# facebookresearch/vilbert-multi-task

Hardware: NVIDIA H100
Metric: (region,token) pairs/sec fwd+bwd, bert_base_6layer_6conect (higher is better)
Workload: dtype fp16

## Files before the change

include/vilbert_b200.h:

```cpp
#ifndef VILBERT_B200_H_
#define VILBERT_B200_H_

#include <stddef.h>
#include <stdint.h>

#ifdef __cplusplus
extern "C" {
#endif

typedef int vb_status;
enum {
  VB_OK = 0,
  VB_ERR_INVALID = 1,
  VB_ERR_UNSUPPORTED = 2,
  VB_ERR_CUDA = 3
};

enum { VB_ACT_NONE = 0, VB_ACT_GELU = 1, VB_ACT_RELU = 2, VB_ACT_DGELU = 3 };

typedef struct vb_dropout_site {
  const uint32_t* step;
  uint32_t site;
  float p;
} vb_dropout_site;
// ... 29 lines not shown
  int64_t ld_out_bf16;
  void* out_pre;
  int64_t ld_out_pre;
  int32_t atomic_out;
  float* out_colsum;
  vb_dropout_site dropout;
  int32_t split_k;
  int32_t block_n;
  int32_t max_ctas;
  void* dbg_timeline;
  int32_t a_fp16, b_fp16, out_fp16;
  const void* A_lo;
  const void* B_lo;
  void* out_lo;
  void* out_b16;
} vb_gemm_args;

vb_status vb_gemm_bf16(const vb_gemm_args* args, void* stream);

vb_status vb_gemm_plan(const vb_gemm_args* args, int32_t sm_count, int32_t* block_n, int32_t* split_k);

typedef struct vb_attn_args {
  int32_t B, H, Nq, Nk, D;
  const void* Q; int64_t ldq;
  const void* K; int64_t ldk;
  const void* V; int64_t ldv;
  const float* mask;
  float scale;
  void* O; int64_t ldo;
  float* lse;
  const void* dO; int64_t lddo;
  void* dQ; int64_t lddq;
  void* dK; int64_t lddk;
  void* dV; int64_t lddv;
  float* delta;
// ... 263 lines not shown
```

vilbert-multi-task_b200/_lib.py:

```python
import ctypes as C
import os
import re
from collections import namedtuple

import torch

_HERE = os.path.dirname(os.path.abspath(__file__))
LIB_PATH = os.path.join(_HERE, "libvilbert_b200.so")
HEADER_PATH = os.path.normpath(os.path.join(_HERE, "..", "include", "vilbert_b200.h"))


class VBError(RuntimeError):
    pass


class DropoutSite(C.Structure):

    _fields_ = [("step", C.c_void_p), ("site", C.c_uint32), ("p", C.c_float)]


class Dropout(DropoutSite):

    _fields_ = [("row_map", C.c_void_p)]

# ... 4 lines not shown
        ("M", C.c_int32), ("N", C.c_int32), ("K", C.c_int32),
        ("A", C.c_void_p), ("lda", C.c_int64), ("a_mn_major", C.c_int32),
        ("B", C.c_void_p), ("ldb", C.c_int64), ("b_mn_major", C.c_int32),
        ("alpha", C.c_float),
        ("bias", C.c_void_p),
        ("residual", C.c_void_p), ("ld_res", C.c_int64),
        ("aux", C.c_void_p), ("ld_aux", C.c_int64),
        ("act", C.c_int32),
        ("out_f32", C.c_void_p), ("ld_out_f32", C.c_int64),
        ("out_bf16", C.c_void_p), ("ld_out_bf16", C.c_int64),
        ("out_pre", C.c_void_p), ("ld_out_pre", C.c_int64),
        ("atomic_out", C.c_int32), ("out_colsum", C.c_void_p), ("dropout", DropoutSite), ("split_k", C.c_int32), ("block_n", C.c_int32), ("max_ctas", C.c_int32),
        ("dbg_timeline", C.c_void_p),
        ("a_fp16", C.c_int32), ("b_fp16", C.c_int32), ("out_fp16", C.c_int32),
        ("A_lo", C.c_void_p), ("B_lo", C.c_void_p), ("out_lo", C.c_void_p), ("out_b16", C.c_void_p),
    ]


class AttnArgs(C.Structure):

    _fields_ = [
        ("B", C.c_int32), ("H", C.c_int32), ("Nq", C.c_int32), ("Nk", C.c_int32), ("D", C.c_int32),
        ("Q", C.c_void_p), ("ldq", C.c_int64), ("K", C.c_void_p), ("ldk", C.c_int64), ("V", C.c_void_p), ("ldv", C.c_int64),
        ("mask", C.c_void_p), ("scale", C.c_float),
        ("O", C.c_void_p), ("ldo", C.c_int64), ("lse", C.c_void_p),
        ("dO", C.c_void_p), ("lddo", C.c_int64), ("dQ", C.c_void_p), ("lddq", C.c_int64),
        ("dK", C.c_void_p), ("lddk", C.c_int64), ("dV", C.c_void_p), ("lddv", C.c_int64),
        ("delta", C.c_void_p),
        ("dbias_q", C.c_void_p), ("dbias_k", C.c_void_p), ("dbias_v", C.c_void_p),
        ("dropout", DropoutSite),
# ... 131 lines not shown
```

vilbert-multi-task_b200/csrc/vb_gemm.cu:

```cuda
#include <cuda.h>
#include <cuda_bf16.h>
#include <cuda_runtime.h>
#include <stdint.h>

#include <type_traits>

#include "vb_internal.h"
#include "vb_ptx.cuh"

namespace vb {

constexpr int BM = 128;
constexpr int BK = 64;
constexpr int UK = 16;
constexpr int CONSUMER_WARPS = 8;
constexpr int GEMM_THREADS = 128 + CONSUMER_WARPS * 32;
constexpr int EPI_ROWS = 16;
constexpr int EPI_PS = EPI_ROWS / 4;
constexpr int STAGING_BYTES_PER_WARP = EPI_ROWS * 32 * 4;
__device__ __forceinline__ int stg_off(int row, int col) { return row * 32 + ((((col >> 2) ^ (row & 7)) << 2) | (col & 3)); }

template <int BN>
struct GemmCfg {
  static constexpr int A_BYTES = BM * BK * 2;
// ... 212 lines not shown
  }
  wgmma_commit();
}

template <int NR>
__device__ __forceinline__ void stage_chunk(const float (&d)[NR], int c4, float* stg, int lane) {
  const int r0 = lane >> 2, c0 = 2 * (lane & 3);
#pragma unroll
  for (int ii = 0; ii < 4; ++ii) {
    const int i = c4 * 4 + ii;
    *reinterpret_cast<float2*>(stg + stg_off(r0, ii * 8 + c0)) = make_float2(d[4 * i], d[4 * i + 1]);
    *reinterpret_cast<float2*>(stg + stg_off(r0 + 8, ii * 8 + c0)) = make_float2(d[4 * i + 2], d[4 * i + 3]);
  }
}

template <int BN, int EPI, int OUT16>
__global__ void __launch_bounds__(GEMM_THREADS, 1)
gemm_wgmma_kernel(const __grid_constant__ CUtensorMap tmap_a, const __grid_constant__ CUtensorMap tmap_b,
                  const __grid_constant__ CUtensorMap tmap_a_lo, const __grid_constant__ CUtensorMap tmap_b_lo,
                  const __grid_constant__ GemmKernelParams p) {
  using Cfg = GemmCfg<BN>;
  constexpr int NUM_STAGES = Cfg::NUM_STAGES;

  extern __shared__ __align__(1024) uint8_t smem[];
  if ((smem_u32(smem) & 1023u) != 0) __trap();
  uint8_t* smem_tiles = smem;
  float* staging = reinterpret_cast<float*>(smem + NUM_STAGES * Cfg::STAGE_BYTES);
  uint64_t* bars = reinterpret_cast<uint64_t*>(smem + NUM_STAGES * Cfg::STAGE_BYTES + CONSUMER_WARPS * STAGING_BYTES_PER_WARP);
  uint64_t* full_bar = bars;
  uint64_t* empty_bar = bars + NUM_STAGES;
// ... 12 lines not shown
      mbar_init(smem_u32(&full_bar[s]), 1);
      mbar_init(smem_u32(&empty_bar[s]), CONSUMER_WARPS);
    }
    fence_mbar_init();
  }
  __syncthreads();
  pdl_entry();
  if (threadIdx.x == 0) VB_DBG(1);

  const int group = blockIdx.x;
  const int num_groups = gridDim.x;
  const int total_work = p.num_m_blocks * p.num_n_blocks * p.split_k;

  if (warp_idx < 4) setmaxnreg_dec<40>();
  if (warp_idx == 0) {
    int stage = 0;
    uint32_t phase = 0;
    for (int w = group; w < total_work; w += num_groups) {
      const int split = w % p.split_k;
      const int t2 = w / p.split_k;
      const int m_blk = t2 % p.num_m_blocks;
      const int n_blk = t2 / p.num_m_blocks;
      const int kb0 = split * p.k_blocks_per_split;
      const int kb1 = min(kb0 + p.k_blocks_per_split, p.num_k_blocks);
      auto issue_loads = [&](const CUtensorMap* tma_a, const CUtensorMap* tma_b, int kb) {
        mbar_wait(smem_u32(&empty_bar[stage]), phase ^ 1);
        const uint32_t sa = smem_u32(smem_tiles + stage * Cfg::STAGE_BYTES);
        const uint32_t sb = sa + Cfg::A_BYTES;
        const uint32_t fb = smem_u32(&full_bar[stage]);
        mbar_arrive_expect_tx(fb, Cfg::STAGE_BYTES);
        if (p.a_mn) {
#pragma unroll
          for (int j = 0; j < BM / 64; ++j) tma_load_2d(sa + j * (BK * 128), tma_a, m_blk * BM + j * 64, kb * BK, fb);
        } else {
          tma_load_2d(sa, tma_a, kb * BK, m_blk * BM, fb);
        }
        if (p.b_mn) {
#pragma unroll
          for (int j = 0; j < BN / 64; ++j) tma_load_2d(sb + j * (BK * 128), tma_b, n_blk * BN + j * 64, kb * BK, fb);
        } else {
          tma_load_2d(sb, tma_b, kb * BK, n_blk * BN, fb);
        }
      };
      for (int kbv = kb0; kbv < kb1; ++kbv) {
        if (elect_one()) {
          if (p.npass == 1) {
            issue_loads(&tmap_a, &tmap_b, kbv);
          } else {
            const int ps = kbv / p.real_k_blocks;
            const int sel = p.pass_sel[ps];
            issue_loads((sel & 1) ? &tmap_a_lo : &tmap_a, (sel & 2) ? &tmap_b_lo : &tmap_b, kbv - ps * p.real_k_blocks);
          }
          if (kbv == kb0 && w == group) VB_DBG(2);
        }
        __syncwarp();
        if (++stage == NUM_STAGES) { stage = 0; phase ^= 1; }
      }
    }
  } else if (warp_idx >= 4) {
    setmaxnreg_inc<232>();
    const int cw = warp_idx - 4;
    const int wg = cw >> 2;
    float* stg = staging + cw * (EPI_ROWS * 32);
    const int rr = lane >> 3;
    const int cc = (lane & 7) * 4;
    const uint32_t a_off = wg * (64 * 128);
    auto release = [&](int s) {
      __syncwarp();
      if (lane == 0) mbar_arrive(smem_u32(&empty_bar[s]));
    };
    float acc[BN / 2];
    int stage = 0;
    uint32_t phase = 0;
// ... 26 lines not shown
        case 1: kloop(std::integral_constant<int, 1>{}); break;
        case 2: kloop(std::integral_constant<int, 2>{}); break;
        case 3: kloop(std::integral_constant<int, 3>{}); break;
        case 4: kloop(std::integral_constant<int, 4>{}); break;
        case 5: kloop(std::integral_constant<int, 5>{}); break;
        case 6: kloop(std::integral_constant<int, 6>{}); break;
        default: kloop(std::integral_constant<int, 7>{}); break;
      }
      wgmma_wait<0>();
#pragma unroll
      for (int i = 0; i < BN / 2; ++i) reg_fence(acc[i]);
      if (prev >= 0) release(prev);
      if (w == group && threadIdx.x == 128) VB_DBG(5);

      const int m_base = m_blk * BM + wg * 64 + (cw & 3) * EPI_ROWS;
      const bool rows_full = (m_base + EPI_ROWS <= p.M);
      if (m_base < p.M) {
        constexpr int NC = BN / 32;
#pragma unroll 1
        for (int c = 0; c < NC; ++c) {
          const int n_chunk = n_blk * BN + c * 32;
          if (n_chunk >= p.N) break;
          const bool fast = (EPI != EPI_GENERIC) && p.fast_ok && rows_full && (n_chunk + 32 <= p.N);
          const int n = n_chunk + cc;
          float4 resv[EPI_PS];
          uint2 auxv[EPI_PS];
          float4 b4 = make_float4(0.f, 0.f, 0.f, 0.f);
          if (fast) {
            if (EPI == EPI_F32 && p.residual) {
#pragma unroll
              for (int ps = 0; ps < EPI_PS; ++ps) {
                const float* src = p.residual + (long long)(m_base + ps * 4 + rr) * p.ld_res + n;
                if (p.vec_res) resv[ps] = *reinterpret_cast<const float4*>(src);
                else resv[ps] = make_float4(src[0], src[1], src[2], src[3]);
              }
            }
            if (EPI == EPI_DGELU) {
#pragma unroll
              for (int ps = 0; ps < EPI_PS; ++ps)
                auxv[ps] = *reinterpret_cast<const uint2*>(p.aux + (long long)(m_base + ps * 4 + rr) * p.ld_aux + n);
            }
            if (p.bias) b4 = *reinterpret_cast<const float4*>(p.bias + n);
          }
#pragma unroll
          for (int c2 = 0; c2 < NC; ++c2)
            if (c2 == c) stage_chunk(acc, c2, stg, lane);
          __syncwarp();
          if (EPI == EPI_PARTIAL) {
            if (fast) epi_fast_chunk<EPI, OUT16>(p, stg, m_base + split * p.M, n, rr, cc, resv, auxv, b4);
            else      epi_partial_chunk(p, stg, m_base, n, rr, cc, (long long)split * p.M);
          }
          else if (EPI == EPI_F32 && p.act == VB_ACT_RELU && fast) epi_pool_chunk(p, stg, m_base, n, rr, cc, b4);
          else if (fast) epi_fast_chunk<EPI, OUT16>(p, stg, m_base, n, rr, cc, resv, auxv, b4);
          else           epi_generic_chunk(p, stg, m_base, n, rr, cc);
          __syncwarp();
        }
      }
      if (w == group && threadIdx.x == 128) VB_DBG(6);
    }
  }

  if (threadIdx.x == 0) { VB_DBG(7); VB_DBG_NS(9); }
#undef VB_DBG
#undef VB_DBG_NS
}

typedef CUresult (*PFN_encodeTiled)(CUtensorMap*, CUtensorMapDataType, cuuint32_t, void*, const cuuint64_t*,
                                    const cuuint64_t*, const cuuint32_t*, const cuuint32_t*,
                                    CUtensorMapInterleave, CUtensorMapSwizzle, CUtensorMapL2promotion,
                                    CUtensorMapFloatOOBfill);

static PFN_encodeTiled get_encode_fn() {
  static PFN_encodeTiled fn = nullptr;
// ... 49 lines not shown
      if (out16 == 2) return launch_gemm<BN, EPI_BF16, 2>(tm, p, work, max_ctas, stream);
      if (out16 == 3) return launch_gemm<BN, EPI_BF16, 3>(tm, p, work, max_ctas, stream);
      return launch_gemm<BN, EPI_BF16, 0>(tm, p, work, max_ctas, stream);
    case EPI_GELU:
      if (out16 == 1) return launch_gemm<BN, EPI_GELU, 1>(tm, p, work, max_ctas, stream);
      if (out16 == 2) return launch_gemm<BN, EPI_GELU, 2>(tm, p, work, max_ctas, stream);
      if (out16 == 3) return launch_gemm<BN, EPI_GELU, 3>(tm, p, work, max_ctas, stream);
      return launch_gemm<BN, EPI_GELU, 0>(tm, p, work, max_ctas, stream);
    case EPI_DGELU: return launch_gemm<BN, EPI_DGELU>(tm, p, work, max_ctas, stream);
    case EPI_ATOMIC: return launch_gemm<BN, EPI_ATOMIC>(tm, p, work, max_ctas, stream);
    case EPI_PARTIAL: return launch_gemm<BN, EPI_PARTIAL>(tm, p, work, max_ctas, stream);
    default: return launch_gemm<BN, EPI_GENERIC>(tm, p, work, max_ctas, stream);
  }
}

static inline bool aligned(const void* p, size_t a) { return (reinterpret_cast<uintptr_t>(p) % a) == 0; }

static int choose_config(const vb_gemm_args* a, int max_ctas, int* bn_out, int* split_out) {
  const int num_m = (a->M + BM - 1) / BM;
  const int num_k = (a->K + BK - 1) / BK * (1 + (a->A_lo ? 1 : 0) + (a->B_lo ? 1 : 0));
  if (a->block_n != 0 && a->block_n != 128 && a->block_n != 256) return set_error(VB_ERR_INVALID, "vb_gemm_bf16: block_n must be 0, 128 or 256");
  if (a->split_k > 1 && (!a->atomic_out || a->act != VB_ACT_NONE || a->bias || a->residual || a->out_colsum))
    return set_error(VB_ERR_INVALID, "vb_gemm_bf16: split_k > 1 needs atomic_out and a plain epilogue");
  const bool can_split = a->atomic_out && a->act == VB_ACT_NONE && !a->bias && !a->residual && !a->out_colsum;
  long long epi_base = 9000;
  if (a->atomic_out) epi_base = 3000;
  else if (a->act == VB_ACT_GELU || a->act == VB_ACT_DGELU) epi_base = 4200;
  else if (a->act == VB_ACT_NONE && a->out_f32 && !a->out_bf16) epi_base = a->residual ? 4800 : 3000;
  else if (a->act == VB_ACT_NONE && a->out_bf16 && !a->out_f32) epi_base = 3000;
  int bn = 128, split_k = 1;
  {
    long long best = -1;
    static const int split_cand[] = {1, 2, 3, 4, 5, 6, 8, 10, 12, 16, 24, 32};
// ... 5 lines not shown
      const long long tiles = (long long)num_m * ((a->N + w - 1) / w);
      for (int sc : split_cand) {
        if (a->split_k > 0 && sc != 1) break;
        int sp = a->split_k > 0 ? a->split_k : sc;
        if (sp > 1 && !can_split) break;
        if (sp > num_k) { if (a->split_k > 0) sp = num_k; else break; }
        const long long kps_ = (num_k + sp - 1) / sp;
        sp = (int)((num_k + kps_ - 1) / kps_);
        const long long rounds = (tiles * sp + max_ctas - 1) / max_ctas;
        const long long ml = kps_ * t_kb;
        const long long c = 3000 + rounds * (ml + epi);
        if (best < 0 || c < best) { best = c; bn = w; split_k = sp; }
      }
    }
    if (best < 0) return set_error(VB_ERR_INVALID, "vb_gemm_bf16: no tile configuration for block_n=%d split_k=%d", a->block_n, a->split_k);
  }
  *bn_out = bn; *split_out = split_k;
  return VB_OK;
}

}

extern "C" vb_status vb_gemm_bf16(const vb_gemm_args* a, void* stream_) {
  using namespace vb;
  cudaStream_t stream = static_cast<cudaStream_t>(stream_);
  if (!a) return set_error(VB_ERR_INVALID, "vb_gemm_bf16: null args");
  if (a->M <= 0 || a->N <= 0 || a->K <= 0) return set_error(VB_ERR_INVALID, "vb_gemm_bf16: empty problem %dx%dx%d", a->M, a->N, a->K);
  if (!a->A || !a->B) return set_error(VB_ERR_INVALID, "vb_gemm_bf16: null operand");
  if ((a->lda % 8) || (a->ldb % 8) || !aligned(a->A, 16) || !aligned(a->B, 16))
    return set_error(VB_ERR_INVALID, "vb_gemm_bf16: operands need ld %% 8 == 0 and 16-byte aligned bases (lda=%lld ldb=%lld)",
// ... 8 lines not shown
  if ((a->A_lo && !aligned(a->A_lo, 16)) || (a->B_lo && !aligned(a->B_lo, 16)))
    return set_error(VB_ERR_INVALID, "vb_gemm_bf16: A_lo / B_lo must be 16-byte aligned");
  if ((a->out_lo || a->out_b16) && !a->out_bf16) return set_error(VB_ERR_INVALID, "vb_gemm_bf16: out_lo / out_b16 need out_bf16");
  if ((a->a_fp16 != 0) != (a->b_fp16 != 0))
    return set_error(VB_ERR_UNSUPPORTED, "vb_gemm_bf16: A and B must have the same 16-bit format (wgmma takes one operand type for both)");
  int dev_sms = 0, cc = 0;
  if (int s = vb_device_info(&dev_sms, &cc)) return s;
  if (cc != 90) return set_error(VB_ERR_UNSUPPORTED, "vb_gemm_bf16: needs an sm_90 device (found sm_%d)", cc);

  const int num_m = (a->M + BM - 1) / BM;
  const int real_k = (a->K + BK - 1) / BK;
  const int npass = 1 + (a->A_lo ? 1 : 0) + (a->B_lo ? 1 : 0);
  const int num_k = real_k * npass;
  int max_ctas = a->max_ctas > 0 ? a->max_ctas : dev_sms;

  int bn = 128, split_k = 1;
  if (int st = choose_config(a, max_ctas, &bn, &split_k)) return st;
  const int num_n = (a->N + bn - 1) / bn;
  const int kps = (num_k + split_k - 1) / split_k;

  GemmKernelParams p;
  p.M = a->M; p.N = a->N; p.K = a->K;
  p.num_m_blocks = num_m; p.num_n_blocks = num_n; p.num_k_blocks = num_k;
  p.real_k_blocks = real_k; p.npass = npass;
  p.pass_sel[0] = 0; p.pass_sel[1] = a->A_lo ? 1 : 2; p.pass_sel[2] = 2;
  p.out_fp16 = a->out_fp16 ? 1 : 0;
  p.out_lo = static_cast<__nv_bfloat16*>(a->out_lo);
  p.out_b16 = static_cast<__nv_bfloat16*>(a->out_b16);
  p.split_k = split_k; p.k_blocks_per_split = kps;
  p.alpha = a->alpha;
  p.bias = a->bias;
  p.residual = a->residual; p.ld_res = a->ld_res;
// ... 28 lines not shown
  for (int i = 0; i < 4; ++i) {
    const bool is_a = (i & 1) == 0;
    const void* ptr = is_a ? (i < 2 ? a->A : a->A_lo) : (i < 2 ? a->B : a->B_lo);
    if (!ptr) { tm[i] = tm[i - 2]; continue; }
    if (is_a) {
      if (a->a_mn_major) st = make_tmap(&tm[i], ptr, (uint64_t)a->M, (uint64_t)a->K, (uint64_t)a->lda, 64, BK);
      else               st = make_tmap(&tm[i], ptr, (uint64_t)a->K, (uint64_t)a->M, (uint64_t)a->lda, BK, BM);
    } else {
      if (a->b_mn_major) st = make_tmap(&tm[i], ptr, (uint64_t)a->N, (uint64_t)a->K, (uint64_t)a->ldb, 64, BK);
      else               st = make_tmap(&tm[i], ptr, (uint64_t)a->K, (uint64_t)a->N, (uint64_t)a->ldb, BK, (uint32_t)bn);
    }
    if (st) return st;
  }

  const long long total_work = (long long)num_m * num_n * split_k;
  int epi = EPI_GENERIC;
  const bool no_extra = !a->out_colsum;
  const bool has_drop = p.drop.ctr != nullptr;
  if (a->atomic_out == VB_GEMM_PARTIALS) {
    if (a->act != VB_ACT_NONE || a->bias || a->residual || !no_extra || has_drop || a->split_k != split_k)
      return set_error(VB_ERR_INVALID, "vb_gemm_bf16: VB_GEMM_PARTIALS needs a plain epilogue and split_k as vb_gemm_plan resolves it "
                       "(asked %d, resolved %d)", a->split_k, split_k);
    epi = EPI_PARTIAL; p.fast_ok = p.vec_f32;
  } else if (a->atomic_out) {
    if (a->act == VB_ACT_NONE && !a->bias && !a->residual && no_extra && !has_drop) { epi = EPI_ATOMIC; p.fast_ok = p.vec_f32; }
  } else if (a->act == VB_ACT_GELU) {
    if (a->out_pre && !a->residual && no_extra && !has_drop && (a->out_bf16 || a->out_f32)) {
      epi = EPI_GELU; p.fast_ok = p.vec_pre && (!a->out_bf16 || p.vec_bf16) && (!a->out_f32 || p.vec_f32);
    }
  } else if (a->act == VB_ACT_DGELU) {
    if (a->out_bf16 && !a->out_f32 && !a->residual && !a->bias && !has_drop) { epi = EPI_DGELU; p.fast_ok = p.vec_bf16 && p.vec_aux; }
  } else if (a->act == VB_ACT_RELU) {
    if (a->out_f32 && no_extra && !a->residual && !has_drop) { epi = EPI_F32; p.fast_ok = p.vec_f32 && (!a->out_bf16 || p.vec_bf16); }
  } else if (a->act == VB_ACT_NONE) {
    if (a->out_f32 && !a->out_bf16 && no_extra) { epi = EPI_F32; p.fast_ok = 1; }
    else if (a->out_bf16 && !a->out_f32 && !a->residual && no_extra && !has_drop) { epi = EPI_BF16; p.fast_ok = p.vec_bf16; }
  }
  int out16 = 0;
  if (epi == EPI_BF16 || epi == EPI_GELU) {
    if ((a->out_lo || a->out_b16) && !a->out_fp16) epi = EPI_GENERIC;
    else out16 = a->out_lo ? 3 : (a->out_fp16 ? (a->out_b16 ? 2 : 1) : 0);
  } else if (epi == EPI_DGELU && (a->out_fp16 || a->out_lo || a->out_b16)) {
    epi = EPI_GENERIC;
  }
  if (bn == 256) return launch_gemm_epi<256>(epi, out16, tm, p, total_work, max_ctas, stream);
  return launch_gemm_epi<128>(epi, out16, tm, p, total_work, max_ctas, stream);
}

extern "C" vb_status vb_gemm_plan(const vb_gemm_args* a, int32_t sm_count_, int32_t* block_n, int32_t* split_k) {
  using namespace vb;
  if (!a || !block_n || !split_k) return set_error(VB_ERR_INVALID, "vb_gemm_plan: null argument");
  if (a->M <= 0 || a->N <= 0 || a->K <= 0) return set_error(VB_ERR_INVALID, "vb_gemm_plan: empty problem %dx%dx%d", a->M, a->N, a->K);
  int sms = sm_count_;
  if (sms <= 0) {
    int cc = 0;
    if (int s = vb_device_info(&sms, &cc)) return s;
  }
  const int max_ctas = a->max_ctas > 0 ? a->max_ctas : sms;
  int bn, sp;
  if (int s = choose_config(a, max_ctas, &bn, &sp)) return s;
  *block_n = bn; *split_k = sp;
  return VB_OK;
}
```

vilbert-multi-task_b200/engine.py:

```python
import bisect
import dataclasses
import math
import warnings
import zlib
from collections import Counter, OrderedDict, namedtuple

import torch

from . import _lib as L

F32, BF16, F16, I64 = torch.float32, torch.bfloat16, torch.float16, torch.int64
PRECISIONS = ("fp16", "fp32", "bf16")
BASE_FEATURE_SIZE, BASE_REGION_CLASSES = 2048, 1601
BASE_HEAD_NAMES = ("vil_prediction", "vil_logit", "vil_binary_prediction", "vision_prediction", "vision_logit", "linguisic_prediction",
                   "linguisic_logit")
BASE_BERT_OUT_NAMES = ("sequence_output", "pooled_output")
INPUT_GRAD_NAMES = ("input_imgs", "image_loc")
PACKED_HEADS = ("vil_prediction", "vil_prediction_gqa", "vil_logit", "vil_binary_prediction", "vil_tri_prediction", "vision_logit")
RETRIEVAL_SCORE_HEADS = {"vl": "vil_logit", "pretraining": "seq_relationship_score"}
PACK_REFUSED_CONFIG = ("in_batch_pairs", "fast_mode", "dynamic_attention", "visualization")
PACKED_MASKED_LOGIT = -10000.0


def pack_capacity(count, padded_rows):
# ... 1013 lines not shown
        else:
            self._check_operands((), (A, B, out_bf16))
        g.M, g.N, g.K = M, N, K
        g.A, g.lda, g.a_mn_major = L.arg(A), lda, a_mn
        g.B, g.ldb, g.b_mn_major = L.arg(B), ldb, b_mn
        g.alpha = alpha
        g.bias = L.arg(bias)
        g.residual, g.ld_res = L.arg(residual), ld_res
        g.aux, g.ld_aux = L.arg(aux), ld_aux
        g.act = act
        g.out_f32, g.ld_out_f32 = L.arg(out_f32), ld_of
        g.out_bf16, g.ld_out_bf16 = L.arg(out_bf16), ld_ob
        g.out_pre, g.ld_out_pre = L.arg(out_pre), ld_op
        g.atomic_out, g.split_k, g.block_n, g.max_ctas = atomic, split_k, 0, (0 if fwd else self.spec.bwd_gemm_max_ctas)
        g.out_colsum = L.arg(None if self.det else out_colsum)
        if dropout is not None:
            g.dropout = dropout
        self._keep.append(g)
        if self.det and atomic:
            g.atomic_out, g.split_k = L.VB_GEMM_PARTIALS, 0
            bn, sp = L.C.c_int32(), L.C.c_int32()
            L.check(self.lib.vb_gemm_plan(L.C.byref(g), 132 if self.dev.type != "cuda" else 0, L.C.byref(bn), L.C.byref(sp)),
                    "vb_gemm_plan")
            if sp.value == 1:
                g.atomic_out, g.split_k = 1, 1
                self.emit(self.lib.vb_gemm_bf16, g)
                return
            if ld_of != N:
                raise L.VBError(f"deterministic split-K GEMM needs a dense output (ld {ld_of} != N {N})")
            ws = self.det_ws(sp.value * M * N)
# ... 1858 lines not shown
```

Measured before the change: 12.79 million.

## Add ping-pong warpgroup GEMM schedule with cost-model auto selection

Adds a ping-pong GEMM kernel in which the two consumer warpgroups work on alternate tiles, so one warpgroup's epilogue runs while the other issues WGMMA. Named barriers order the two groups. A cycle-based cost model picks between cooperative and ping-pong per GEMM, and the engine asks for AUTO unless deterministic mode is on. It also prefetches the next chunk's epilogue inputs (residual, aux, bias) during the current chunk. The risks are a poor choice from the hand-fitted cost constants, and extra register pressure from keeping two 64x128 accumulators per warpgroup.

New measurement: 12.77 million, median of 6. About the same (-0.1%).

```diff
diff --git a/include/vilbert_b200.h b/include/vilbert_b200.h
--- a/include/vilbert_b200.h
+++ b/include/vilbert_b200.h
@@ -67,11 +67,15 @@
   const void* B_lo;
   void* out_lo;
   void* out_b16;
+  int32_t schedule;
 } vb_gemm_args;
 
+enum { VB_GEMM_SCHED_COOPERATIVE = 0, VB_GEMM_SCHED_PINGPONG = 1, VB_GEMM_SCHED_AUTO = 2 };
+
 vb_status vb_gemm_bf16(const vb_gemm_args* args, void* stream);
 
 vb_status vb_gemm_plan(const vb_gemm_args* args, int32_t sm_count, int32_t* block_n, int32_t* split_k);
+vb_status vb_gemm_plan_schedule(const vb_gemm_args* args, int32_t sm_count, int32_t* block_n, int32_t* split_k, int32_t* schedule);
 
 typedef struct vb_attn_args {
   int32_t B, H, Nq, Nk, D;
diff --git a/vilbert-multi-task_b200/_lib.py b/vilbert-multi-task_b200/_lib.py
--- a/vilbert-multi-task_b200/_lib.py
+++ b/vilbert-multi-task_b200/_lib.py
@@ -42,6 +42,7 @@
         ("dbg_timeline", C.c_void_p),
         ("a_fp16", C.c_int32), ("b_fp16", C.c_int32), ("out_fp16", C.c_int32),
         ("A_lo", C.c_void_p), ("B_lo", C.c_void_p), ("out_lo", C.c_void_p), ("out_b16", C.c_void_p),
+        ("schedule", C.c_int32),
     ]
 
 
diff --git a/vilbert-multi-task_b200/csrc/vb_gemm.cu b/vilbert-multi-task_b200/csrc/vb_gemm.cu
--- a/vilbert-multi-task_b200/csrc/vb_gemm.cu
+++ b/vilbert-multi-task_b200/csrc/vb_gemm.cu
@@ -250,6 +250,106 @@
   }
 }
 
+template <int BN>
+__device__ __forceinline__ void gemm_produce(const CUtensorMap* tmap_a, const CUtensorMap* tmap_b, const CUtensorMap* tmap_a_lo,
+                                             const CUtensorMap* tmap_b_lo, const GemmKernelParams& p, uint8_t* smem_tiles,
+                                             uint64_t* full_bar, uint64_t* empty_bar, int group, int num_groups, int total_work) {
+  using Cfg = GemmCfg<BN>;
+  int stage = 0;
+  uint32_t phase = 0;
+  for (int w = group; w < total_work; w += num_groups) {
+    const int split = w % p.split_k;
+    const int t2 = w / p.split_k;
+    const int m_blk = t2 % p.num_m_blocks;
+    const int n_blk = t2 / p.num_m_blocks;
+    const int kb0 = split * p.k_blocks_per_split;
+    const int kb1 = min(kb0 + p.k_blocks_per_split, p.num_k_blocks);
+    auto issue_loads = [&](const CUtensorMap* tma_a, const CUtensorMap* tma_b, int kb) {
+      mbar_wait(smem_u32(&empty_bar[stage]), phase ^ 1);
+      const uint32_t sa = smem_u32(smem_tiles + stage * Cfg::STAGE_BYTES);
+      const uint32_t sb = sa + Cfg::A_BYTES;
+      const uint32_t fb = smem_u32(&full_bar[stage]);
+      mbar_arrive_expect_tx(fb, Cfg::STAGE_BYTES);
+      if (p.a_mn) {
+#pragma unroll
+        for (int j = 0; j < BM / 64; ++j) tma_load_2d(sa + j * (BK * 128), tma_a, m_blk * BM + j * 64, kb * BK, fb);
+      } else {
+        tma_load_2d(sa, tma_a, kb * BK, m_blk * BM, fb);
+      }
+      if (p.b_mn) {
+#pragma unroll
+        for (int j = 0; j < BN / 64; ++j) tma_load_2d(sb + j * (BK * 128), tma_b, n_blk * BN + j * 64, kb * BK, fb);
+      } else {
+        tma_load_2d(sb, tma_b, kb * BK, n_blk * BN, fb);
+      }
+    };
+    for (int kbv = kb0; kbv < kb1; ++kbv) {
+      if (elect_one()) {
+        if (p.npass == 1) {
+          issue_loads(tmap_a, tmap_b, kbv);
+        } else {
+          const int ps = kbv / p.real_k_blocks;
+          const int sel = p.pass_sel[ps];
+          issue_loads((sel & 1) ? tmap_a_lo : tmap_a, (sel & 2) ? tmap_b_lo : tmap_b, kbv - ps * p.real_k_blocks);
+        }
+        if (kbv == kb0 && w == group && p.dbg) p.dbg[blockIdx.x * 10 + 2] = clock64();
+      }
+      __syncwarp();
+      if (++stage == Cfg::NUM_STAGES) { stage = 0; phase ^= 1; }
+    }
+  }
+}
+
+struct ChunkIn {
+  float4 resv[EPI_PS];
+  uint2 auxv[EPI_PS];
+  float4 b4;
+};
+__device__ __forceinline__ bool chunk_fast(const GemmKernelParams& p, int epi, int m_base, int n_chunk) {
+  return epi != EPI_GENERIC && p.fast_ok && m_base + EPI_ROWS <= p.M && n_chunk + 32 <= p.N;
+}
+template <int EPI>
+__device__ __forceinline__ ChunkIn chunk_in(const GemmKernelParams& p, int m_base, int n_chunk, int rr, int cc) {
+  ChunkIn in;
+  in.b4 = make_float4(0.f, 0.f, 0.f, 0.f);
+  if (chunk_fast(p, EPI, m_base, n_chunk)) {
+    const int n = n_chunk + cc;
+    if (EPI == EPI_F32 && p.residual) {
+#pragma unroll
+      for (int ps = 0; ps < EPI_PS; ++ps) {
+        const float* src = p.residual + (long long)(m_base + ps * 4 + rr) * p.ld_res + n;
+        if (p.vec_res) in.resv[ps] = *reinterpret_cast<const float4*>(src);
+        else in.resv[ps] = make_float4(src[0], src[1], src[2], src[3]);
+      }
+    }
+    if (EPI == EPI_DGELU) {
+#pragma unroll
+      for (int ps = 0; ps < EPI_PS; ++ps)
+        in.auxv[ps] = *reinterpret_cast<const uint2*>(p.aux + (long long)(m_base + ps * 4 + rr) * p.ld_aux + n);
+    }
+    if (p.bias) in.b4 = *reinterpret_cast<const float4*>(p.bias + n);
+  }
+  return in;
+}
+
+template <int EPI, int OUT16, typename Prefetch, typename Stage>
+__device__ __forceinline__ void epilogue_chunk(const GemmKernelParams& p, float* stg, int m_base, int n_chunk, int split, int rr, int cc,
+                                               const ChunkIn& in, Prefetch&& prefetch, Stage&& stage) {
+  const bool fast = chunk_fast(p, EPI, m_base, n_chunk);
+  const int n = n_chunk + cc;
+  prefetch();
+  stage();
+  __syncwarp();
+  if (EPI == EPI_PARTIAL) {
+    if (fast) epi_fast_chunk<EPI, OUT16>(p, stg, m_base + split * p.M, n, rr, cc, in.resv, in.auxv, in.b4);
+    else      epi_partial_chunk(p, stg, m_base, n, rr, cc, (long long)split * p.M);
+  }
+  else if (EPI == EPI_F32 && p.act == VB_ACT_RELU && fast) epi_pool_chunk(p, stg, m_base, n, rr, cc, in.b4);
+  else if (fast) epi_fast_chunk<EPI, OUT16>(p, stg, m_base, n, rr, cc, in.resv, in.auxv, in.b4);
+  else           epi_generic_chunk(p, stg, m_base, n, rr, cc);
+  __syncwarp();
+}
+
 template <int BN, int EPI, int OUT16>
 __global__ void __launch_bounds__(GEMM_THREADS, 1)
 gemm_wgmma_kernel(const __grid_constant__ CUtensorMap tmap_a, const __grid_constant__ CUtensorMap tmap_b,
@@ -292,49 +392,7 @@
 
   if (warp_idx < 4) setmaxnreg_dec<40>();
   if (warp_idx == 0) {
-    int stage = 0;
-    uint32_t phase = 0;
-    for (int w = group; w < total_work; w += num_groups) {
-      const int split = w % p.split_k;
-      const int t2 = w / p.split_k;
-      const int m_blk = t2 % p.num_m_blocks;
-      const int n_blk = t2 / p.num_m_blocks;
-      const int kb0 = split * p.k_blocks_per_split;
-      const int kb1 = min(kb0 + p.k_blocks_per_split, p.num_k_blocks);
-      auto issue_loads = [&](const CUtensorMap* tma_a, const CUtensorMap* tma_b, int kb) {
-        mbar_wait(smem_u32(&empty_bar[stage]), phase ^ 1);
-        const uint32_t sa = smem_u32(smem_tiles + stage * Cfg::STAGE_BYTES);
-        const uint32_t sb = sa + Cfg::A_BYTES;
-        const uint32_t fb = smem_u32(&full_bar[stage]);
-        mbar_arrive_expect_tx(fb, Cfg::STAGE_BYTES);
-        if (p.a_mn) {
-#pragma unroll
-          for (int j = 0; j < BM / 64; ++j) tma_load_2d(sa + j * (BK * 128), tma_a, m_blk * BM + j * 64, kb * BK, fb);
-        } else {
-          tma_load_2d(sa, tma_a, kb * BK, m_blk * BM, fb);
-        }
-        if (p.b_mn) {
-#pragma unroll
-          for (int j = 0; j < BN / 64; ++j) tma_load_2d(sb + j * (BK * 128), tma_b, n_blk * BN + j * 64, kb * BK, fb);
-        } else {
-          tma_load_2d(sb, tma_b, kb * BK, n_blk * BN, fb);
-        }
-      };
-      for (int kbv = kb0; kbv < kb1; ++kbv) {
-        if (elect_one()) {
-          if (p.npass == 1) {
-            issue_loads(&tmap_a, &tmap_b, kbv);
-          } else {
-            const int ps = kbv / p.real_k_blocks;
-            const int sel = p.pass_sel[ps];
-            issue_loads((sel & 1) ? &tmap_a_lo : &tmap_a, (sel & 2) ? &tmap_b_lo : &tmap_b, kbv - ps * p.real_k_blocks);
-          }
-          if (kbv == kb0 && w == group) VB_DBG(2);
-        }
-        __syncwarp();
-        if (++stage == NUM_STAGES) { stage = 0; phase ^= 1; }
-      }
-    }
+    gemm_produce<BN>(&tmap_a, &tmap_b, &tmap_a_lo, &tmap_b_lo, p, smem_tiles, full_bar, empty_bar, group, num_groups, total_work);
   } else if (warp_idx >= 4) {
     setmaxnreg_inc<232>();
     const int cw = warp_idx - 4;
@@ -391,49 +449,186 @@
       if (w == group && threadIdx.x == 128) VB_DBG(5);
 
       const int m_base = m_blk * BM + wg * 64 + (cw & 3) * EPI_ROWS;
-      const bool rows_full = (m_base + EPI_ROWS <= p.M);
       if (m_base < p.M) {
         constexpr int NC = BN / 32;
+        ChunkIn cur = chunk_in<EPI>(p, m_base, n_blk * BN, rr, cc), nxt;
 #pragma unroll 1
         for (int c = 0; c < NC; ++c) {
           const int n_chunk = n_blk * BN + c * 32;
           if (n_chunk >= p.N) break;
-          const bool fast = (EPI != EPI_GENERIC) && p.fast_ok && rows_full && (n_chunk + 32 <= p.N);
-          const int n = n_chunk + cc;
-          float4 resv[EPI_PS];
-          uint2 auxv[EPI_PS];
-          float4 b4 = make_float4(0.f, 0.f, 0.f, 0.f);
-          if (fast) {
-            if (EPI == EPI_F32 && p.residual) {
-#pragma unroll
-              for (int ps = 0; ps < EPI_PS; ++ps) {
-                const float* src = p.residual + (long long)(m_base + ps * 4 + rr) * p.ld_res + n;
-                if (p.vec_res) resv[ps] = *reinterpret_cast<const float4*>(src);
-                else resv[ps] = make_float4(src[0], src[1], src[2], src[3]);
-              }
+          epilogue_chunk<EPI, OUT16>(p, stg, m_base, n_chunk, split, rr, cc, cur,
+                                     [&] { if (c + 1 < NC) nxt = chunk_in<EPI>(p, m_base, n_chunk + 32, rr, cc); },
+                                     [&] {
+#pragma unroll
+            for (int c2 = 0; c2 < NC; ++c2)
+              if (c2 == c) stage_chunk(acc, c2, stg, lane);
+          });
+          cur = nxt;
+        }
+      }
+      if (w == group && threadIdx.x == 128) VB_DBG(6);
+    }
+  }
+
+  if (threadIdx.x == 0) { VB_DBG(7); VB_DBG_NS(9); }
+#undef VB_DBG
+#undef VB_DBG_NS
+}
+
+constexpr int PP_BAR_MATH = 1;
+constexpr int PP_BAR_EPI = 3;
+constexpr int PP_BAR_THREADS = 256;
+__device__ __forceinline__ void named_bar_sync(int id) { asm volatile("bar.sync %0, %1;" ::"r"(id), "n"(PP_BAR_THREADS) : "memory"); }
+__device__ __forceinline__ void named_bar_arrive(int id) { asm volatile("bar.arrive %0, %1;" ::"r"(id), "n"(PP_BAR_THREADS) : "memory"); }
+
+template <int F16, int TA, int TB>
+__device__ __forceinline__ void mma_kblock_pp(float (&acc0)[64], float (&acc1)[64], uint32_t sa, uint32_t sb, uint64_t desc_base_a,
+                                              uint64_t desc_base_b, bool accumulate) {
+  wgmma_fence();
+#pragma unroll
+  for (int k = 0; k < BK / UK; ++k) {
+    const uint32_t ka = k * (TA ? 2048 : UK * 2);
+    const uint64_t db = gmma_desc_at(desc_base_b, sb + k * (TB ? 2048 : UK * 2));
+    wgmma_m64n128k16<F16, TA, TB>(acc0, gmma_desc_at(desc_base_a, sa + ka), db, (accumulate || k > 0) ? 1u : 0u);
+    wgmma_m64n128k16<F16, TA, TB>(acc1, gmma_desc_at(desc_base_a, sa + 64 * 128 + ka), db, (accumulate || k > 0) ? 1u : 0u);
+  }
+  wgmma_commit();
+}
+
+template <int EPI, int OUT16>
+__global__ void __launch_bounds__(GEMM_THREADS, 1)
+gemm_pingpong_kernel(const __grid_constant__ CUtensorMap tmap_a, const __grid_constant__ CUtensorMap tmap_b,
+                     const __grid_constant__ CUtensorMap tmap_a_lo, const __grid_constant__ CUtensorMap tmap_b_lo,
+                     const __grid_constant__ GemmKernelParams p) {
+  using Cfg = GemmCfg<128>;
+  constexpr int NUM_STAGES = Cfg::NUM_STAGES;
+
+  extern __shared__ __align__(1024) uint8_t smem[];
+  if ((smem_u32(smem) & 1023u) != 0) __trap();
+  uint8_t* smem_tiles = smem;
+  float* staging = reinterpret_cast<float*>(smem + NUM_STAGES * Cfg::STAGE_BYTES);
+  uint64_t* bars = reinterpret_cast<uint64_t*>(smem + NUM_STAGES * Cfg::STAGE_BYTES + CONSUMER_WARPS * STAGING_BYTES_PER_WARP);
+  uint64_t* full_bar = bars;
+  uint64_t* empty_bar = bars + NUM_STAGES;
+
+  const int warp_idx = threadIdx.x >> 5;
+  const int lane = threadIdx.x & 31;
+#define VB_DBG(slot) do { if (p.dbg) p.dbg[blockIdx.x * 10 + (slot)] = clock64(); } while (0)
+#define VB_DBG_NS(slot) do { if (p.dbg) { unsigned long long t_; asm volatile("mov.u64 %0, %%globaltimer;" : "=l"(t_)); p.dbg[blockIdx.x * 10 + (slot)] = t_; } } while (0)
+  if (threadIdx.x == 0) { VB_DBG(0); VB_DBG_NS(8); }
+
+  if (threadIdx.x == 0) {
+    tma_prefetch_desc(&tmap_a);
+    tma_prefetch_desc(&tmap_b);
+    if (p.npass > 1) { tma_prefetch_desc(&tmap_a_lo); tma_prefetch_desc(&tmap_b_lo); }
+    for (int s = 0; s < NUM_STAGES; ++s) {
+      mbar_init(smem_u32(&full_bar[s]), 1);
+      mbar_init(smem_u32(&empty_bar[s]), 4);
+    }
+    fence_mbar_init();
+  }
+  __syncthreads();
+  pdl_entry();
+  if (threadIdx.x == 0) VB_DBG(1);
+
+  const int group = blockIdx.x;
+  const int num_groups = gridDim.x;
+  const int total_work = p.num_m_blocks * p.num_n_blocks * p.split_k;
+
+  if (warp_idx < 4) setmaxnreg_dec<40>();
+  if (warp_idx == 0) {
+    gemm_produce<128>(&tmap_a, &tmap_b, &tmap_a_lo, &tmap_b_lo, p, smem_tiles, full_bar, empty_bar, group, num_groups, total_work);
+  } else if (warp_idx >= 4) {
+    setmaxnreg_inc<232>();
+    const int cw = warp_idx - 4;
+    const int wg = cw >> 2;
+    float* stg = staging + cw * (EPI_ROWS * 32);
+    const int rr = lane >> 3;
+    const int cc = (lane & 7) * 4;
+    auto release = [&](int s) {
+      __syncwarp();
+      if (lane == 0) mbar_arrive(smem_u32(&empty_bar[s]));
+    };
+    auto item_kblocks = [&](int w) {
+      const int kb0 = (w % p.split_k) * p.k_blocks_per_split;
+      return min(kb0 + p.k_blocks_per_split, p.num_k_blocks) - kb0;
+    };
+    int stage = 0;
+    uint32_t phase = 0;
+    auto advance = [&](int n) {
+      const int t = stage + n;
+      phase ^= (uint32_t)((t / NUM_STAGES) & 1);
+      stage = t % NUM_STAGES;
+    };
+    float acc0[64], acc1[64];
+    const int mma_kind = p.mma_kind;
+    const uint64_t desc_base_a = p.desc_base_a, desc_base_b = p.desc_base_b;
+    if (wg == 1) advance(item_kblocks(group));
+    for (int w = group + wg * num_groups, j = wg; w < total_work; w += 2 * num_groups, j += 2) {
+      const bool has_next = w + num_groups < total_work;
+      const int split = w % p.split_k;
+      const int t2 = w / p.split_k;
+      const int m_blk = t2 % p.num_m_blocks;
+      const int n_blk = t2 / p.num_m_blocks;
+      const int kb0 = split * p.k_blocks_per_split;
+      const int kb1 = min(kb0 + p.k_blocks_per_split, p.num_k_blocks);
+      int prev = -1;
+      if (j > 0) named_bar_sync(PP_BAR_MATH + wg);
+      auto kloop = [&](auto kind) {
+        constexpr int KIND = decltype(kind)::value;
+        for (int kb = kb0; kb < kb1; ++kb) {
+          mbar_wait(smem_u32(&full_bar[stage]), phase);
+          if (kb == kb0 && j == 0 && threadIdx.x == 128) VB_DBG(3);
+          const uint32_t sa = smem_u32(smem_tiles + stage * Cfg::STAGE_BYTES);
+          mma_kblock_pp<(KIND >> 2) & 1, (KIND >> 1) & 1, KIND & 1>(acc0, acc1, sa, sa + Cfg::A_BYTES, desc_base_a, desc_base_b, kb > kb0);
+          wgmma_wait<1>();
+          if (prev >= 0) release(prev);
+          prev = stage;
+          if (++stage == NUM_STAGES) { stage = 0; phase ^= 1; }
+        }
+      };
+      switch (mma_kind) {
+        case 0: kloop(std::integral_constant<int, 0>{}); break;
+        case 1: kloop(std::integral_constant<int, 1>{}); break;
+        case 2: kloop(std::integral_constant<int, 2>{}); break;
+        case 3: kloop(std::integral_constant<int, 3>{}); break;
+        case 4: kloop(std::integral_constant<int, 4>{}); break;
+        case 5: kloop(std::integral_constant<int, 5>{}); break;
+        case 6: kloop(std::integral_constant<int, 6>{}); break;
+        default: kloop(std::integral_constant<int, 7>{}); break;
+      }
+      if (has_next) named_bar_arrive(PP_BAR_MATH + (wg ^ 1));
+      wgmma_wait<0>();
+#pragma unroll
+      for (int i = 0; i < 64; ++i) { reg_fence(acc0[i]); reg_fence(acc1[i]); }
+      if (prev >= 0) release(prev);
+      if (has_next) advance(item_kblocks(w + num_groups));
+      if (j == 0 && threadIdx.x == 128) VB_DBG(5);
+
+      if (j > 0) named_bar_sync(PP_BAR_EPI + wg);
+      auto m_of = [&](int c) { return m_blk * BM + (c >> 2) * 64 + (cw & 3) * EPI_ROWS; };
+      auto n_of = [&](int c) { return n_blk * 128 + (c & 3) * 32; };
+      auto next_of = [&](int c) { return (c + 1 < 8 && n_of(c + 1) >= p.N) ? ((c + 1) | 3) + 1 : c + 1; };
+      ChunkIn cur = chunk_in<EPI>(p, m_of(0), n_of(0), rr, cc), nxt;
+#pragma unroll 1
+      for (int c = 0; c < 8; c = next_of(c)) {
+        const int m_base = m_of(c);
+        if (m_base >= p.M) break;
+        const int cn = next_of(c);
+        epilogue_chunk<EPI, OUT16>(p, stg, m_base, n_of(c), split, rr, cc, cur,
+                                   [&] { if (cn < 8) nxt = chunk_in<EPI>(p, m_of(cn), n_of(cn), rr, cc); },
+                                   [&] {
+#pragma unroll
+          for (int c2 = 0; c2 < 8; ++c2)
+            if (c2 == c) {
+              if (c2 < 4) stage_chunk(acc0, c2, stg, lane);
+              else        stage_chunk(acc1, c2 - 4, stg, lane);
             }
-            if (EPI == EPI_DGELU) {
-#pragma unroll
-              for (int ps = 0; ps < EPI_PS; ++ps)
-                auxv[ps] = *reinterpret_cast<const uint2*>(p.aux + (long long)(m_base + ps * 4 + rr) * p.ld_aux + n);
-            }
-            if (p.bias) b4 = *reinterpret_cast<const float4*>(p.bias + n);
-          }
-#pragma unroll
-          for (int c2 = 0; c2 < NC; ++c2)
-            if (c2 == c) stage_chunk(acc, c2, stg, lane);
-          __syncwarp();
-          if (EPI == EPI_PARTIAL) {
-            if (fast) epi_fast_chunk<EPI, OUT16>(p, stg, m_base + split * p.M, n, rr, cc, resv, auxv, b4);
-            else      epi_partial_chunk(p, stg, m_base, n, rr, cc, (long long)split * p.M);
-          }
-          else if (EPI == EPI_F32 && p.act == VB_ACT_RELU && fast) epi_pool_chunk(p, stg, m_base, n, rr, cc, b4);
-          else if (fast) epi_fast_chunk<EPI, OUT16>(p, stg, m_base, n, rr, cc, resv, auxv, b4);
-          else           epi_generic_chunk(p, stg, m_base, n, rr, cc);
-          __syncwarp();
-        }
-      }
-      if (w == group && threadIdx.x == 128) VB_DBG(6);
+        });
+        cur = nxt;
+      }
+      if (has_next) named_bar_arrive(PP_BAR_EPI + (wg ^ 1));
+      if (j == 0 && threadIdx.x == 128) VB_DBG(6);
     }
   }
 
@@ -513,9 +708,101 @@
   }
 }
 
+template <int EPI, int OUT16 = 0>
+static int launch_gemm_pp(const CUtensorMap* tm, GemmKernelParams& p, long long total_work, int max_ctas, cudaStream_t stream) {
+  using Cfg = GemmCfg<128>;
+  auto kern = gemm_pingpong_kernel<EPI, OUT16>;
+  static bool attr_set = false;
+  if (!attr_set) {
+    cudaError_t e = cudaFuncSetAttribute(kern, cudaFuncAttributeMaxDynamicSharedMemorySize, Cfg::SMEM_BYTES);
+    if (e != cudaSuccess) return set_error(VB_ERR_CUDA, "cudaFuncSetAttribute: %s", cudaGetErrorString(e));
+    attr_set = true;
+  }
+  const int grid = (int)(total_work < max_ctas ? total_work : max_ctas);
+  cudaError_t e = launch_pdl(kern, dim3(grid), dim3(GEMM_THREADS), (size_t)Cfg::SMEM_BYTES, stream, tm[0], tm[1], tm[2], tm[3], p);
+  if (e != cudaSuccess) return set_error(VB_ERR_CUDA, "gemm launch: %s", cudaGetErrorString(e));
+  return VB_OK;
+}
+
+static int launch_gemm_pp_epi(int epi, int out16, const CUtensorMap* tm, GemmKernelParams& p, long long work, int max_ctas,
+                              cudaStream_t stream) {
+  switch (epi) {
+    case EPI_F32: return launch_gemm_pp<EPI_F32>(tm, p, work, max_ctas, stream);
+    case EPI_BF16:
+      if (out16 == 1) return launch_gemm_pp<EPI_BF16, 1>(tm, p, work, max_ctas, stream);
+      if (out16 == 2) return launch_gemm_pp<EPI_BF16, 2>(tm, p, work, max_ctas, stream);
+      if (out16 == 3) return launch_gemm_pp<EPI_BF16, 3>(tm, p, work, max_ctas, stream);
+      return launch_gemm_pp<EPI_BF16, 0>(tm, p, work, max_ctas, stream);
+    case EPI_GELU:
+      if (out16 == 1) return launch_gemm_pp<EPI_GELU, 1>(tm, p, work, max_ctas, stream);
+      if (out16 == 2) return launch_gemm_pp<EPI_GELU, 2>(tm, p, work, max_ctas, stream);
+      if (out16 == 3) return launch_gemm_pp<EPI_GELU, 3>(tm, p, work, max_ctas, stream);
+      return launch_gemm_pp<EPI_GELU, 0>(tm, p, work, max_ctas, stream);
+    case EPI_DGELU: return launch_gemm_pp<EPI_DGELU>(tm, p, work, max_ctas, stream);
+    case EPI_ATOMIC: return launch_gemm_pp<EPI_ATOMIC>(tm, p, work, max_ctas, stream);
+    case EPI_PARTIAL: return launch_gemm_pp<EPI_PARTIAL>(tm, p, work, max_ctas, stream);
+    default: return set_error(VB_ERR_UNSUPPORTED, "vb_gemm_bf16: the ping-pong schedule has no generic epilogue");
+  }
+}
+
 static inline bool aligned(const void* p, size_t a) { return (reinterpret_cast<uintptr_t>(p) % a) == 0; }
 
-static int choose_config(const vb_gemm_args* a, int max_ctas, int* bn_out, int* split_out) {
+static int epilogue_form(const vb_gemm_args* a, int* out16_out) {
+  int epi = EPI_GENERIC;
+  const bool no_extra = !a->out_colsum;
+  const bool has_drop = a->dropout.step && a->dropout.p > 0.f;
+  if (a->atomic_out == VB_GEMM_PARTIALS) {
+    epi = EPI_PARTIAL;
+  } else if (a->atomic_out) {
+    if (a->act == VB_ACT_NONE && !a->bias && !a->residual && no_extra && !has_drop) epi = EPI_ATOMIC;
+  } else if (a->act == VB_ACT_GELU) {
+    if (a->out_pre && !a->residual && no_extra && !has_drop && (a->out_bf16 || a->out_f32)) epi = EPI_GELU;
+  } else if (a->act == VB_ACT_DGELU) {
+    if (a->out_bf16 && !a->out_f32 && !a->residual && !a->bias && !has_drop) epi = EPI_DGELU;
+  } else if (a->act == VB_ACT_RELU) {
+    if (a->out_f32 && no_extra && !a->residual && !has_drop) epi = EPI_F32;
+  } else if (a->act == VB_ACT_NONE) {
+    if (a->out_f32 && !a->out_bf16 && no_extra) epi = EPI_F32;
+    else if (a->out_bf16 && !a->out_f32 && !a->residual && no_extra && !has_drop) epi = EPI_BF16;
+  }
+  int out16 = 0;
+  if (epi == EPI_BF16 || epi == EPI_GELU) {
+    if ((a->out_lo || a->out_b16) && !a->out_fp16) epi = EPI_GENERIC;
+    else out16 = a->out_lo ? 3 : (a->out_fp16 ? (a->out_b16 ? 2 : 1) : 0);
+  } else if (epi == EPI_DGELU && (a->out_fp16 || a->out_lo || a->out_b16)) {
+    epi = EPI_GENERIC;
+  }
+  *out16_out = out16;
+  return epi;
+}
+
+enum { FORM_F32, FORM_F32_SCALAR, FORM_BF16, FORM_GELU, FORM_DGELU, FORM_ATOMIC, FORM_COUNT };
+static const long long EPI_COOP128[FORM_COUNT] = {4800, 26000,     5500,  7500,  11000, 4100};
+static const long long EPI_COOP256[FORM_COUNT] = {13500, 52000,    10500, 24000, 25000, 11400};
+static const long long EPI_PP[FORM_COUNT]      = {12000, 23000,    13000, 20000, 25000, 9800};
+
+static int epilogue_cost_form(const vb_gemm_args* a, int epi) {
+  if (epi == EPI_ATOMIC || epi == EPI_PARTIAL) return FORM_ATOMIC;
+  if (epi == EPI_GELU) return FORM_GELU;
+  if (epi == EPI_DGELU) return FORM_DGELU;
+  if (epi == EPI_BF16) return FORM_BF16;
+  return (a->ld_out_f32 % 4 != 0) ? FORM_F32_SCALAR : FORM_F32;
+}
+
+static long long measured_cycles(const vb_gemm_args* a, int form, bool pingpong, int bn, int split, int num_m, int num_k, int max_ctas) {
+  const bool mn = a->a_mn_major || a->b_mn_major;
+  const long long tiles = (long long)num_m * ((a->N + bn - 1) / bn) * split;
+  const long long rounds = (tiles + max_ctas - 1) / max_ctas;
+  const long long kps = (num_k + split - 1) / split;
+  if (!pingpong) {
+    const long long kb = bn == 256 ? (mn ? 1300 : 1060) : (mn ? 750 : 640);
+    return 3000 + rounds * (kps * kb + (bn == 256 ? EPI_COOP256 : EPI_COOP128)[form]);
+  }
+  const long long ml = kps * (mn ? 1100 : 860), e = EPI_PP[form];
+  return 3000 + rounds * (ml > e ? ml : e) + (ml > e ? e : ml);
+}
+
+static int choose_config(const vb_gemm_args* a, int max_ctas, int* bn_out, int* split_out, int* sched_out) {
   const int num_m = (a->M + BM - 1) / BM;
   const int num_k = (a->K + BK - 1) / BK * (1 + (a->A_lo ? 1 : 0) + (a->B_lo ? 1 : 0));
   if (a->block_n != 0 && a->block_n != 128 && a->block_n != 256) return set_error(VB_ERR_INVALID, "vb_gemm_bf16: block_n must be 0, 128 or 256");
@@ -551,6 +838,25 @@
       }
     }
     if (best < 0) return set_error(VB_ERR_INVALID, "vb_gemm_bf16: no tile configuration for block_n=%d split_k=%d", a->block_n, a->split_k);
+    *sched_out = VB_GEMM_SCHED_COOPERATIVE;
+    if (a->schedule == VB_GEMM_SCHED_COOPERATIVE) { *bn_out = bn; *split_out = split_k; return VB_OK; }
+
+    int out16;
+    const int epi = epilogue_form(a, &out16);
+    const bool pp_ok = num_k == (a->K + BK - 1) / BK && epi != EPI_GENERIC && a->block_n != 256;
+    if (a->schedule == VB_GEMM_SCHED_PINGPONG && !pp_ok)
+      return set_error(VB_ERR_UNSUPPORTED, "vb_gemm_bf16: the ping-pong schedule needs single-pass operands, a specialised epilogue "
+                       "and block_n 0 or 128");
+    if (a->schedule != VB_GEMM_SCHED_PINGPONG && a->schedule != VB_GEMM_SCHED_AUTO)
+      return set_error(VB_ERR_INVALID, "vb_gemm_bf16: schedule must be VB_GEMM_SCHED_COOPERATIVE, _PINGPONG or _AUTO");
+    if (pp_ok) {
+      const int form = epilogue_cost_form(a, epi);
+      if (a->schedule == VB_GEMM_SCHED_PINGPONG ||
+          measured_cycles(a, form, true, 128, split_k, num_m, num_k, max_ctas) < measured_cycles(a, form, false, bn, split_k, num_m, num_k, max_ctas)) {
+        bn = 128;
+        *sched_out = VB_GEMM_SCHED_PINGPONG;
+      }
+    }
   }
   *bn_out = bn; *split_out = split_k;
   return VB_OK;
@@ -589,8 +895,8 @@
   const int num_k = real_k * npass;
   int max_ctas = a->max_ctas > 0 ? a->max_ctas : dev_sms;
 
-  int bn = 128, split_k = 1;
-  if (int st = choose_config(a, max_ctas, &bn, &split_k)) return st;
+  int bn = 128, split_k = 1, sched = VB_GEMM_SCHED_COOPERATIVE;
+  if (int st = choose_config(a, max_ctas, &bn, &split_k, &sched)) return st;
   const int num_n = (a->N + bn - 1) / bn;
   const int kps = (num_k + split_k - 1) / split_k;
 
@@ -649,42 +955,30 @@
   }
 
   const long long total_work = (long long)num_m * num_n * split_k;
-  int epi = EPI_GENERIC;
-  const bool no_extra = !a->out_colsum;
-  const bool has_drop = p.drop.ctr != nullptr;
-  if (a->atomic_out == VB_GEMM_PARTIALS) {
-    if (a->act != VB_ACT_NONE || a->bias || a->residual || !no_extra || has_drop || a->split_k != split_k)
-      return set_error(VB_ERR_INVALID, "vb_gemm_bf16: VB_GEMM_PARTIALS needs a plain epilogue and split_k as vb_gemm_plan resolves it "
-                       "(asked %d, resolved %d)", a->split_k, split_k);
-    epi = EPI_PARTIAL; p.fast_ok = p.vec_f32;
-  } else if (a->atomic_out) {
-    if (a->act == VB_ACT_NONE && !a->bias && !a->residual && no_extra && !has_drop) { epi = EPI_ATOMIC; p.fast_ok = p.vec_f32; }
-  } else if (a->act == VB_ACT_GELU) {
-    if (a->out_pre && !a->residual && no_extra && !has_drop && (a->out_bf16 || a->out_f32)) {
-      epi = EPI_GELU; p.fast_ok = p.vec_pre && (!a->out_bf16 || p.vec_bf16) && (!a->out_f32 || p.vec_f32);
-    }
-  } else if (a->act == VB_ACT_DGELU) {
-    if (a->out_bf16 && !a->out_f32 && !a->residual && !a->bias && !has_drop) { epi = EPI_DGELU; p.fast_ok = p.vec_bf16 && p.vec_aux; }
-  } else if (a->act == VB_ACT_RELU) {
-    if (a->out_f32 && no_extra && !a->residual && !has_drop) { epi = EPI_F32; p.fast_ok = p.vec_f32 && (!a->out_bf16 || p.vec_bf16); }
-  } else if (a->act == VB_ACT_NONE) {
-    if (a->out_f32 && !a->out_bf16 && no_extra) { epi = EPI_F32; p.fast_ok = 1; }
-    else if (a->out_bf16 && !a->out_f32 && !a->residual && no_extra && !has_drop) { epi = EPI_BF16; p.fast_ok = p.vec_bf16; }
-  }
   int out16 = 0;
-  if (epi == EPI_BF16 || epi == EPI_GELU) {
-    if ((a->out_lo || a->out_b16) && !a->out_fp16) epi = EPI_GENERIC;
-    else out16 = a->out_lo ? 3 : (a->out_fp16 ? (a->out_b16 ? 2 : 1) : 0);
-  } else if (epi == EPI_DGELU && (a->out_fp16 || a->out_lo || a->out_b16)) {
-    epi = EPI_GENERIC;
-  }
+  const int epi = epilogue_form(a, &out16);
+  switch (epi) {
+    case EPI_PARTIAL:
+      if (a->act != VB_ACT_NONE || a->bias || a->residual || a->out_colsum || p.drop.ctr || a->split_k != split_k)
+        return set_error(VB_ERR_INVALID, "vb_gemm_bf16: VB_GEMM_PARTIALS needs a plain epilogue and split_k as vb_gemm_plan resolves it "
+                         "(asked %d, resolved %d)", a->split_k, split_k);
+      p.fast_ok = p.vec_f32; break;
+    case EPI_ATOMIC: p.fast_ok = p.vec_f32; break;
+    case EPI_GELU: p.fast_ok = p.vec_pre && (!a->out_bf16 || p.vec_bf16) && (!a->out_f32 || p.vec_f32); break;
+    case EPI_DGELU: p.fast_ok = p.vec_bf16 && p.vec_aux; break;
+    case EPI_F32: p.fast_ok = a->act == VB_ACT_RELU ? (p.vec_f32 && (!a->out_bf16 || p.vec_bf16)) : 1; break;
+    case EPI_BF16: p.fast_ok = p.vec_bf16; break;
+    default: break;
+  }
+  if (sched == VB_GEMM_SCHED_PINGPONG) return launch_gemm_pp_epi(epi, out16, tm, p, total_work, max_ctas, stream);
   if (bn == 256) return launch_gemm_epi<256>(epi, out16, tm, p, total_work, max_ctas, stream);
   return launch_gemm_epi<128>(epi, out16, tm, p, total_work, max_ctas, stream);
 }
 
-extern "C" vb_status vb_gemm_plan(const vb_gemm_args* a, int32_t sm_count_, int32_t* block_n, int32_t* split_k) {
+extern "C" vb_status vb_gemm_plan_schedule(const vb_gemm_args* a, int32_t sm_count_, int32_t* block_n, int32_t* split_k,
+                                           int32_t* schedule) {
   using namespace vb;
-  if (!a || !block_n || !split_k) return set_error(VB_ERR_INVALID, "vb_gemm_plan: null argument");
+  if (!a || !block_n || !split_k || !schedule) return set_error(VB_ERR_INVALID, "vb_gemm_plan: null argument");
   if (a->M <= 0 || a->N <= 0 || a->K <= 0) return set_error(VB_ERR_INVALID, "vb_gemm_plan: empty problem %dx%dx%d", a->M, a->N, a->K);
   int sms = sm_count_;
   if (sms <= 0) {
@@ -692,8 +986,13 @@
     if (int s = vb_device_info(&sms, &cc)) return s;
   }
   const int max_ctas = a->max_ctas > 0 ? a->max_ctas : sms;
-  int bn, sp;
-  if (int s = choose_config(a, max_ctas, &bn, &sp)) return s;
-  *block_n = bn; *split_k = sp;
+  int bn, sp, sched;
+  if (int s = choose_config(a, max_ctas, &bn, &sp, &sched)) return s;
+  *block_n = bn; *split_k = sp; *schedule = sched;
   return VB_OK;
 }
+
+extern "C" vb_status vb_gemm_plan(const vb_gemm_args* a, int32_t sm_count_, int32_t* block_n, int32_t* split_k) {
+  int32_t schedule;
+  return vb_gemm_plan_schedule(a, sm_count_, block_n, split_k, &schedule);
+}
diff --git a/vilbert-multi-task_b200/engine.py b/vilbert-multi-task_b200/engine.py
--- a/vilbert-multi-task_b200/engine.py
+++ b/vilbert-multi-task_b200/engine.py
@@ -1051,6 +1051,7 @@
         g.out_pre, g.ld_out_pre = L.arg(out_pre), ld_op
         g.atomic_out, g.split_k, g.block_n, g.max_ctas = atomic, split_k, 0, (0 if fwd else self.spec.bwd_gemm_max_ctas)
         g.out_colsum = L.arg(None if self.det else out_colsum)
+        g.schedule = L.VB_GEMM_SCHED_COOPERATIVE if self.det else L.VB_GEMM_SCHED_AUTO
         if dropout is not None:
             g.dropout = dropout
         self._keep.append(g)
```
